# Lainshower/debiasing-multi-modal

Hardware: AMD Instinct MI355X
Metric: images/sec (embed+adapter step), CLIP-RN50 224px bs=1024 (higher is better)
Workload: dtype f32; 1 GPU; CLIP-RN50 224px encode_image + adapter(1024-128-1024) CE/SGD step, 1024 images/GPU, global batch 1024 (the metric's configuration, CLIP-RN50 224px bs=1024 on one GPU); global_batch=1024, batch_per_gpu=1024, parallelism=dp1, collective=none

## Files before the change

### debiasing-multi-modal_amd/_lib.py

```python
import ctypes
import glob
import os
import subprocess
from ctypes import c_double, c_float, c_int, c_int64, c_size_t, c_void_p

_HERE = os.path.dirname(os.path.abspath(__file__))
CSRC = os.path.join(_HERE, "csrc")
LIB_PATH = os.environ.get("DBMM_LIB") or os.path.join(_HERE, "libdbmm_hip.so")
INCLUDE = os.path.join(os.path.dirname(_HERE), "include")

_lib = None


def sources():
    return sorted(glob.glob(os.path.join(CSRC, "*.hip")))


KERNEL_SOURCES = (
    ("igemm_", ("igemm_f32.hip", "igemm_epilogue.inc", "common.h")),
    ("bottleneck_chain_kernel", ("bottleneck_chain.hip", "common.h")),
    ("bottleneck_chain8_kernel", ("bottleneck_chain8.hip", "common.h")),
    ("conv3x3_c32_kernel", ("conv_patch.hip", "common.h")),
    ("gemm_pair_8ph_kernel", ("gemm_pair_8ph.hip", "gemm_pair_8ph_epilogue.inc", "persistent_tiles.h", "common.h")),
    ("conv3x3_halo8", ("conv3x3_halo8.hip", "conv3x3_halo8_epilogue.inc", "persistent_tiles.h", "common.h")),
# ... 101 lines not shown
    "dbmm_bottleneck_chain_pool_f16": [_P, _P, _P, _P, _P, _P, _P, _P, _P, _P, _P, _L, _L, _L, _L, _L, _L, _P],
    "dbmm_bottleneck_chain_dual_f16": [_P, _P, _P, _P, _P, _P, _P, _P, _P, _P, _P, _P, _L, _L, _L, _L, _L, _P],
    "dbmm_conv3x3_bn_relu_f16": [_P, _P, _P, _P, _P, _L, _L, _L, _L, _L, _I, _P],
    "dbmm_conv_stem_s2_f16": [_P, _I, _P, _P, _P, _L, _L, _L, _L, _P],
    "dbmm_conv1x1_res_pool_f16": [_P, _P, _P, _P, _P, _P, _P, _L, _L, _L, _L, _L, _P],
    "dbmm_conv_stem_s2_bn_f16": [_P, _I, _P, _P, _P, _P, _L, _L, _L, _L, _P],
    "dbmm_avgpool2_f16": [_P, _P, _L, _L, _L, _L, _P],
    "dbmm_im2col_patch_f16": [_P, _I, _P, _L, _L, _L, _L, _P],
    "dbmm_vit_tokens_f16": [_P, _P, _P, _P, _L, _L, _L, _P],
    "dbmm_embed_gather_f16": [_P, _P, _P, _P, _L, _L, _L, _L, _P],
    "dbmm_gather_eot_f16": [_P, _P, _P, _L, _L, _L, _P],
    "dbmm_cast_f32_f16": [_P, _P, _L, _P],
    "dbmm_conv3x3_c32_bn_relu_x2": [_P, _P, _P, _I, _P, _P, _P, _P, _L, _L, _L, _L, _L, _I, _P],
    "dbmm_bottleneck_block_chain_x2": [_P, _P, _P, _I, _P, _P, _P, _I, _P, _P, _P, _P, _P, _P, _P, _P, _P, _P, _I, _P, _P, _P, _P,
                                       _L, _L, _L, _L, _L, _L, _P],
    "dbmm_gemm_bias_act_x3": [_P, _L, _P, _P, _L, _P, _P, _L, _P, _L, _L, _L, _L, _F, _I, _P, _Z, _P],
    "dbmm_gemm_batched": [_P, _L, _L, _I, _P, _L, _L, _I, _P, _L, _P, _L, _L, _L, _L, _L, _L, _F, _I, _P],
    "dbmm_gemm_pair_8ph": [_P, _L, _P, _P, _I, _L, _P, _P, _P, _L, _P, _L, _P, _L, _L, _L, _F, _I, _P],
    "dbmm_conv_stem_s2": [_P, _P, _P, _P, _P, _L, _L, _L, _L, _P],
    "dbmm_avgpool2d": [_P, _P, _L, _L, _L, _L, _L, _P],
    "dbmm_workspace_bytes_attnpool": [_L, _L, _L],
    "dbmm_attnpool": [_P, _P, _P, _P, _P, _P, _P, _P, _P, _L, _L, _L, _L, _L, _P, _Z, _P],
    "dbmm_attnpool_x": [_P, _I, _P, _P, _P, _P, _P, _P, _P, _P, _L, _L, _L, _L, _L, _P, _Z, _P],
    "dbmm_layernorm": [_P, _L, _P, _P, _P, _L, _L, _L, _F, _P, _P],
    "dbmm_mha_core": [_P, _P, _L, _L, _L, _L, _I, _P],
    "dbmm_mha_core_x2": [_P, _P, _P, _L, _L, _L, _L, _I, _P],
    "dbmm_embed_gather": [_P, _P, _P, _P, _L, _L, _L, _L, _P],
    "dbmm_im2col_patch": [_P, _P, _P, _L, _L, _L, _P],
    "dbmm_vit_tokens": [_P, _P, _P, _P, _L, _L, _L, _P],
    "dbmm_gather_eot": [_P, _P, _P, _L, _L, _L, _P],
# ... 147 lines not shown
```

### debiasing-multi-modal_amd/clip/model.py

```python
import os
import re
from collections import OrderedDict
from typing import Tuple, Union

import numpy as np
import torch
from torch import nn

from .. import ops



class _ConvW(nn.Module):
    def __init__(self, cin, cout, k):
        super().__init__()
        self.weight = nn.Parameter(torch.empty(cout, cin, k, k))


class _BNParams(nn.Module):
    def __init__(self, c):
        super().__init__()
        self.weight = nn.Parameter(torch.ones(c))
        self.bias = nn.Parameter(torch.zeros(c))
        self.register_buffer("running_mean", torch.zeros(c))
# ... 58 lines not shown

def _fold_bn(conv_w, bn):
    s = bn.weight.double() / torch.sqrt(bn.running_var.double() + bn.eps)
    w = conv_w.double() * s.reshape(-1, 1, 1, 1)
    b = bn.bias.double() - bn.running_mean.double() * s
    return w, b


def _conv_bn(conv, bn):
    w, b = _fold_bn(conv.weight, bn)
    scale = bn.weight.detach().double() / torch.sqrt(bn.running_var.detach().double() + bn.eps)
    return _pack_conv(w, b, raw=conv.weight.detach().float(), scale=scale)


_PLAN_OPTIONS = {"conv_split": ("f16", ("f16", "bf16", "off")), "conv_k_order": ("chunk32", ("chunk32", "tap")),
                 "fuse_ds": (1, (0, 1)), "fuse_chain": (1, (0, 1)), "fuse_conv2": (1, (0, 1)), "seam_pool": (2, (0, 1, 2))}
_opt = {}
_opt_version = [0]


def set_plan_option(name, value):
    default, allowed = _PLAN_OPTIONS[name]
    if isinstance(default, int):
        value = int(value)
    if value not in allowed:
        raise ValueError(f"plan option {name}: {value!r} not in {allowed}")
    old = _opt.get(name, default)
    _opt[name] = value
    _opt_version[0] += 1
    return old

# ... 240 lines not shown
                else:
                    out, oam = conv(x, am, e["c1"], None, 1, 0, ops.ACT_RELU)
                nxt = blocks[bi] if bi < len(blocks) else None
                if (e["stride"] == 1 and track and _opt["fuse_chain"] and _opt["fuse_conv2"] and nxt is not None and nxt["stride"] == 1
                        and all(c["sc"] is not None and c["ph"] is not None for c in (e["c2"], e["c3"], nxt["c1"]))
                        and ("ds" not in e or ("dual" in e and _opt["fuse_ds"]))):
                    ndsl = 3 if "ds" in e else 2
                    x_am, y1_am = amax[slot[0] + 1:slot[0] + 2], amax[slot[0] + ndsl:slot[0] + ndsl + 1]
                    dual = dict(a2=x, a2_absmax=am, ds=e["ds"], ratio=e["dual"]["ratio"], bias=e["dual"]["bias"]) if "ds" in e else None
                    r = ops.bottleneck_block_chain(out, oam, e["c2"], e["c3"], nxt["c1"], residual=None if dual else x, dual=dual,
                                                   x_absmax=x_am, y1n_absmax=y1_am)
                    if r is not None:
                        slot[0] += ndsl + 1
                        x, am, x_pooled, y1_next = r[0], x_am, None, (r[1], y1_am)
                        continue
                if e["stride"] == 2:
                    out, oam = conv(out, oam, e["c2"], None, 3, 1, ops.ACT_RELU, pool=2)
                else:
                    out, oam = conv(out, oam, e["c2"], None, 3, 1, ops.ACT_RELU)
                    if e["stride"] > 1:
                        out = ops.avgpool2d(out, e["stride"])
                identity = x
                fused = None
                if "ds" in e:
                    if e["stride"] > 1:
                        identity = x_pooled if (x_pooled is not None and e["stride"] == 2) else ops.avgpool2d(x, e["stride"])
                    nxt = blocks[bi] if bi < len(blocks) else None
                    if ("dual" in e and track and _opt["fuse_ds"] and _opt["fuse_chain"] and e["stride"] == 1 and nxt is not None
                            and nxt["c1"]["sc"] is not None and nxt["c1"]["ph"] is not None and "ds" not in nxt):
                        x_am, y1_am = amax[slot[0]:slot[0] + 1], amax[slot[0] + 2:slot[0] + 3]
# ... 325 lines not shown
```

### debiasing-multi-modal_amd/csrc/bottleneck_chain.hip

```cpp
#include <stdlib.h>
#include "common.h"

namespace {

struct ChainP {
    const float* a; const float* a_absmax;
    const u16* w3; int w3_exp; const float* sc3; const float* b3;
    const float* res; float* x; float* xp; float* x_absmax;
    const u16* w1; int w1_exp; const float* sc1; const float* b1;
    float* y1; float* y1_absmax;
    int M, N;
    int Ho, Wo;
    const float* a2; const float* a2_absmax; const u16* wd; const float* ratio;
    const u16* w2; int w2_exp; const float* sc2; const float* b2;
    int H, W;
};

template <int RH>
__device__ __forceinline__ int swz(int row) { return RH == 32 ? ((row >> 2) & 3) : (RH == 64 ? ((row >> 1) & 7) : (row & 15)); }

constexpr int BM = 128;

template <int K, int P>
struct ChainGeo {
    static constexpr int BNS = K == 64 ? 64 : 32;
    static constexpr int SLROW = BNS + 4;
    static constexpr int R1_BYTES = BM * SLROW * 4 > 2 * BM * 64 * 2 ? BM * SLROW * 4 : 2 * BM * 64 * 2;
    static constexpr int W3_BYTES = BNS * K * 2;
    static constexpr int W1_BYTES = P * BNS * 2;
    static constexpr int LDS_BYTES = R1_BYTES + W3_BYTES + W1_BYTES;
// ... 8 lines not shown
}

constexpr int C2_SROWS = 132, C2_PLANE = C2_SROWS * 32;
constexpr int C2_W2P = 104;
template <int K>
struct Conv2Geo {
    static constexpr int W2_OFF = 2 * C2_PLANE;
    static constexpr int GROUP_BYTES = (2 * C2_PLANE * 2 + K * C2_W2P * 2 + 255) / 256 * 256;
    static constexpr int NST = K == 64 ? 2 : 1;
    static constexpr int Z_OFF = NST * GROUP_BYTES;
    static constexpr int BYTES = Z_OFF + 256;
    static constexpr int STAGE_BYTES = BM * 68 * 4;
};
constexpr int cmax(int a, int b) { return a > b ? a : b; }

template <int K, int P, int POOL, int DUAL = 0, int CONV2 = 0>
__global__ __launch_bounds__(256, 2) void bottleneck_chain_kernel(const ChainP p) {
    static_assert(!DUAL || K == 64, "dual-source variant: layer-1 geometry (K = K2 = 64)");
    static_assert(!CONV2 || !POOL, "the conv2 phase walks pixels in standard order");
    static_assert(K == 64 || K == 128, "conv3 reduction depth: 64 (layer 1) or 128 (layer 2)");
    static_assert(P == 64 || P == 128, "conv1' width");
    using G = ChainGeo<K, P>;
    constexpr int BNS = G::BNS, SLROW = G::SLROW;
    constexpr int KS = K / 16, TN3 = BNS / 32, TN1 = P / 32;
    constexpr int LDS_TOTAL = cmax(G::LDS_BYTES + (DUAL ? BNS * 64 * 2 : 0), CONV2 ? cmax(Conv2Geo<K>::BYTES, Conv2Geo<K>::STAGE_BYTES) : 0);
    __shared__ __attribute__((aligned(256))) unsigned char lds_raw[LDS_TOTAL];
    u16* Ay = (u16*)lds_raw;
    float* slab = (float*)lds_raw;
    u16* W3b = (u16*)(lds_raw + G::R1_BYTES);
    u16* W1b = (u16*)(lds_raw + G::R1_BYTES + G::W3_BYTES);
    u16* Wdb = (u16*)(lds_raw + G::R1_BYTES + G::W3_BYTES + G::W1_BYTES);

    const int tid = threadIdx.x, lane = tid & 63, wave = tid >> 6;
    const int fr = lane & 31, fh = lane >> 5;
    const int m0 = xcd_remap(blockIdx.x, gridDim.x) * BM;
    const int NT = p.N / BNS;

    const int g0 = row_pixel<POOL>(p, m0);
    const long long Mll = p.M;
    const __amdgpu_buffer_rsrc_t rsA = desc(p.a, Mll * K * 4, (long long)g0 * K * 4);
    const __amdgpu_buffer_rsrc_t rsR = DUAL ? desc(p.a2, Mll * 64 * 4, (long long)g0 * 64 * 4)
                                            : desc(p.res, Mll * p.N * 4, (long long)g0 * p.N * 4);
    const __amdgpu_buffer_rsrc_t rsX = desc(p.x, POOL == 2 ? 0 : Mll * p.N * 4, (long long)g0 * p.N * 4);
    const __amdgpu_buffer_rsrc_t rsY = desc(p.y1, Mll * P * 4, (long long)g0 * P * 4);
    __amdgpu_buffer_rsrc_t rsXP = rsX;
    if constexpr (POOL) rsXP = desc(p.xp, (Mll >> 2) * p.N * 4, (long long)(m0 >> 2) * p.N * 4);

    unsigned gx[4], gy[4];
#pragma unroll
    for (int t = 0; t < 4; ++t) {
        const int m = m0 + wave * 32 + 8 * t + 4 * fh;
        const int dp = row_pixel<POOL>(p, m) - g0;
        gx[t] = m < p.M ? (unsigned)dp * (unsigned)(p.N * 4) + (unsigned)(fr * 4) : OOR;
        gy[t] = m < p.M ? (unsigned)dp * (unsigned)(P * 4) + (unsigned)(fr * 4) : OOR;
    }
    auto qpix = [&](int q) { return POOL ? (q >> 1) * p.Wo + (q & 1) : q; };

    constexpr int CPR3 = K / 8, RPP3 = 256 / CPR3, W3LD = BNS * CPR3 / 256;
    constexpr int CPR1 = BNS / 8, RPP1 = 256 / CPR1, W1LD = P * CPR1 / 256;
    static_assert(W3LD >= 1 && W1LD >= 1, "weight slabs smaller than one pass of the workgroup");
    const int wc3 = tid % CPR3, wr3 = tid / CPR3, wc1 = tid % CPR1, wr1 = tid / CPR1;
    u32x4 w3r[W3LD], w1r[W1LD], wdr[DUAL ? W3LD : 1];
    auto load_w = [&](int nt) {
#pragma unroll
        for (int j = 0; j < W3LD; ++j) {
            w3r[j] = *(const u32x4*)(p.w3 + (size_t)(nt * BNS + wr3 + RPP3 * j) * K + wc3 * 8);
            if constexpr (DUAL) wdr[j] = *(const u32x4*)(p.wd + (size_t)(nt * BNS + wr3 + RPP3 * j) * 64 + wc3 * 8);
        }
#pragma unroll
        for (int j = 0; j < W1LD; ++j)
            w1r[j] = *(const u32x4*)(p.w1 + (size_t)(wr1 + RPP1 * j) * p.N + nt * BNS + wc1 * 8);
    };
    auto store_w = [&]() {
#pragma unroll
        for (int j = 0; j < W3LD; ++j) {
            const int row = wr3 + RPP3 * j;
            *(u32x4*)(W3b + row * K + ((wc3 ^ swz<K>(row)) << 3)) = w3r[j];
// ... 11 lines not shown
        if constexpr (DUAL) return;
#pragma unroll
        for (int j = 0; j < TN3; ++j)
#pragma unroll
            for (int r = 0; r < 16; ++r)
                rr[j][r] = __builtin_bit_cast(float, __builtin_amdgcn_raw_buffer_load_b32(
                    rsR, gx[r >> 2], (unsigned)((nt * BNS + j * 32) * 4 + qpix(r & 3) * p.N * 4), 0));
    };
    load_res(0);
    u32x4 af[KS][2], af2[DUAL ? 4 : 1][2];
    bool first_pass = true;
    auto stage_issue = [&](const __amdgpu_buffer_rsrc_t& rs, int ldk, int k0, f32x4 (&q)[8]) {
        const int lc = tid & 15, lr = tid >> 4;
#pragma unroll
        for (int i = 0; i < 8; ++i) {
            const int row = lr + 16 * i, m = m0 + row;
            const unsigned off = m < p.M ? (unsigned)(row_pixel<POOL>(p, m) - g0) * (unsigned)(ldk * 4) + lc * 16u : OOR;
            q[i] = __builtin_bit_cast(f32x4, __builtin_amdgcn_raw_buffer_load_b128(rs, off, (unsigned)(k0 * 4), 0));
        }
    };
    auto stage_finish = [&](const f32x4 (&q)[8], float sc, u32x4 (*dst)[2]) {
        const int lc = tid & 15, lr = tid >> 4;
        if (!first_pass) __syncthreads();
#pragma unroll
        for (int i = 0; i < 8; ++i) {
            const int row = lr + 16 * i;
            unsigned hp[2], lp[2];
#pragma unroll
            for (int j = 0; j < 2; ++j) split2h_pair(q[i][2 * j], q[i][2 * j + 1], sc, hp[j], lp[j]);
            const int off = row * 64 + (((lc >> 1) ^ swz<64>(row)) << 3) + ((lc & 1) << 2);
            *(u32x2*)(Ay + off) = (u32x2){hp[0], hp[1]};
            *(u32x2*)(Ay + BM * 64 + off) = (u32x2){lp[0], lp[1]};
// ... 18 lines not shown
    if constexpr (DUAL && CONV2) stage_issue(rsR, 64, 0, q2);
    int s_a;
    if constexpr (!CONV2) {
        s_a = scale_exp(*p.a_absmax);
#pragma unroll
        for (int kp = 0; kp < K / 64; ++kp) stage_pass(rsA, K, kp * 64, pow2f(s_a), af + kp * 4);
    } else {
        using C2 = Conv2Geo<K>;
        constexpr int TN2 = K / 32, NG = (K / 32) * 3, W2LD = (K * 12 + 255) / 256;
        u16* Sp = (u16*)lds_raw;
        constexpr int NST = C2::NST, STH = C2::GROUP_BYTES / 2;
        constexpr int ZLH = C2::Z_OFF / 2;
        if (tid < 16) *(u32x4*)(lds_raw + C2::Z_OFF + tid * 16) = (u32x4){0u, 0u, 0u, 0u};
        const int s_y1 = scale_exp(*p.a_absmax);
        const float y1_sc = pow2f(s_y1);
        const int px0 = m0 - 1 - p.W > 0 ? m0 - 1 - p.W : 0;
        const __amdgpu_buffer_rsrc_t rsS = desc(p.a, Mll * K * 4, (long long)px0 * K * 4);
        const int lc = tid & 7, lr = tid >> 3;
        unsigned s_off[5];
#pragma unroll
        for (int i = 0; i < 5; ++i) {
            const int j = lr + 32 * i;
            s_off[i] = j < 130 ? (unsigned)((m0 - 1 + j - px0) * (K * 4)) + lc * 16u : OOR;
        }
        unsigned fmask = 0;
        {
            const int m = m0 + wave * 32 + fr;
            if (m < p.M) {
                const int hw = p.H * p.W, rem = m - (m / hw) * hw, ho = rem / p.W, wo = rem - ho * p.W;
#pragma unroll
                for (int kh = 0; kh < 3; ++kh)
#pragma unroll
                    for (int kw = 0; kw < 3; ++kw)
                        if (ho + kh - 1 >= 0 && ho + kh - 1 < p.H && wo + kw - 1 >= 0 && wo + kw - 1 < p.W) fmask |= 1u << (kh * 3 + kw);
            }
        }
        f32x4 sq[5];
        u32x4 w2q[W2LD];
        auto load_group = [&](int g) {
            const int sl = g / 3, kh = g - sl * 3;
            const unsigned delta = (unsigned)(((kh - 1) * p.W * K + sl * 32) * 4);
#pragma unroll
            for (int i = 0; i < 5; ++i)
// ... 26 lines not shown
            }
        };
        f32x16 acc2[TN2];
#pragma unroll
        for (int j = 0; j < TN2; ++j)
#pragma unroll
            for (int r = 0; r < 16; ++r) acc2[j][r] = 0.f;
        auto compute_group = [&](int g, int st) {
            const u16* Sps = Sp + st * STH;
            const u16* W2b = Sps + C2::W2_OFF;
            const int zl = ZLH - st * STH;
            const int kh = g % 3;
#pragma unroll
            for (int kw = 0; kw < 3; ++kw) {
                const bool ok = (fmask >> (kh * 3 + kw)) & 1u;
                const int row = wave * 32 + fr + kw;
#pragma unroll
                for (int ks = 0; ks < 2; ++ks) {
                    const int addr = row * 32 + (((2 * ks + fh) ^ swz<32>(row)) << 3);
                    const int a0 = ok ? addr : zl + (addr & 127), a1 = ok ? addr + C2_PLANE : zl + (addr & 127);
                    const u32x4 ah = *(const u32x4*)(Sps + a0), al = *(const u32x4*)(Sps + a1);
                    u32x4 wf[TN2];
#pragma unroll
                    for (int j = 0; j < TN2; ++j) wf[j] = *(const u32x4*)(W2b + (j * 32 + fr) * C2_W2P + kw * 32 + (2 * ks + fh) * 8);
#pragma unroll
                    for (int j = 0; j < TN2; ++j)
                        acc2[j] = __builtin_amdgcn_mfma_f32_32x32x16_f16(__builtin_bit_cast(f16x8, al), __builtin_bit_cast(f16x8, wf[j]), acc2[j], 0, 0, 0);
#pragma unroll
                    for (int j = 0; j < TN2; ++j)
                        acc2[j] = __builtin_amdgcn_mfma_f32_32x32x16_f16(__builtin_bit_cast(f16x8, ah), __builtin_bit_cast(f16x8, wf[j]), acc2[j], 0, 0, 0);
                }
// ... 52 lines not shown
        }
        __syncthreads();
        if constexpr (!DUAL) store_w();
    }
    float dual_dyn = 1.f;
    if constexpr (DUAL) {
        const int s_a2 = scale_exp(*p.a2_absmax);
        if constexpr (CONV2) stage_finish(q2, pow2f(s_a2), af2);
        else stage_pass(rsR, 64, 0, pow2f(s_a2), af2);
        dual_dyn = pow2f(s_a - s_a2);
    }
    __syncthreads();

    float* Ls = slab + wave * (32 * SLROW);
    const float acc3_scale = pow2f(-s_a - p.w3_exp);
    f32x16 acc1[TN1];
#pragma unroll
    for (int j = 0; j < TN1; ++j)
#pragma unroll
        for (int r = 0; r < 16; ++r) acc1[j][r] = 0.f;
    float run_max = 0.f, x_amax = 0.f;
    int s_cur = 0;

    for (int nt = 0; nt < NT; ++nt) {
        const int n0 = nt * BNS;
        if (nt + 1 < NT) load_w(nt + 1);
        f32x16 acc3[TN3];
#pragma unroll
        for (int j = 0; j < TN3; ++j)
#pragma unroll
            for (int r = 0; r < 16; ++r) acc3[j][r] = 0.f;
// ... 37 lines not shown
        }
        float tmax = 0.f;
#pragma unroll
        for (int j = 0; j < TN3; ++j) {
            const int n = n0 + j * 32 + fr;
            const float sv = p.sc3[n] * acc3_scale, bv = p.b3[n];
#pragma unroll
            for (int r = 0; r < 16; ++r) {
                float v = fmaxf(fmaf(acc3[j][r], sv, bv) + (DUAL ? 0.f : rr[j][r]), 0.f);
                if (gx[r >> 2] == OOR) v = 0.f;
                acc3[j][r] = v;
                tmax = fmaxf(tmax, v);
                if constexpr (POOL != 2)
                    __builtin_amdgcn_raw_buffer_store_b32(__builtin_bit_cast(unsigned, v), rsX, gx[r >> 2],
                                                          (unsigned)((n0 + j * 32) * 4 + qpix(r & 3) * p.N * 4), 0);
                Ls[((r & 3) + 8 * (r >> 2) + 4 * fh) * SLROW + j * 32 + fr] = v;
            }
            if constexpr (POOL) {
#pragma unroll
                for (int t = 0; t < 4; ++t) {
                    const float s = (((acc3[j][4 * t] + acc3[j][4 * t + 1]) + acc3[j][4 * t + 2]) + acc3[j][4 * t + 3]) * 0.25f;
                    const int mp = wave * 8 + 2 * t + fh;
                    const unsigned off = gx[t] != OOR ? (unsigned)mp * (unsigned)(p.N * 4) + (unsigned)(fr * 4) : OOR;
                    __builtin_amdgcn_raw_buffer_store_b32(__builtin_bit_cast(unsigned, s), rsXP, off, (unsigned)((n0 + j * 32) * 4), 0);
                }
            }
        }
        if (nt + 1 < NT) load_res(nt + 1);
        tmax = wave_max(tmax);
        x_amax = fmaxf(x_amax, tmax);
        if (tmax > run_max) {
            run_max = tmax;
            const int s_new = scale_exp(run_max);
            if (s_new != s_cur) {
                const float f = pow2f(s_new - s_cur);
#pragma unroll
                for (int j = 0; j < TN1; ++j)
#pragma unroll
                    for (int r = 0; r < 16; ++r) acc1[j][r] *= f;
                s_cur = s_new;
            }
        }
        const float t_sc = pow2f(s_cur);
#pragma unroll
        for (int ks = 0; ks < BNS / 16; ++ks) {
            const f32x4 x0 = *(const f32x4*)(Ls + fr * SLROW + 16 * ks + 8 * fh);
            const f32x4 x1 = *(const f32x4*)(Ls + fr * SLROW + 16 * ks + 8 * fh + 4);
            unsigned h[4], l[4];
            split2h_pair(x0[0], x0[1], t_sc, h[0], l[0]); split2h_pair(x0[2], x0[3], t_sc, h[1], l[1]);
            split2h_pair(x1[0], x1[1], t_sc, h[2], l[2]); split2h_pair(x1[2], x1[3], t_sc, h[3], l[3]);
            const u32x4 ah = {h[0], h[1], h[2], h[3]}, al = {l[0], l[1], l[2], l[3]};
            u32x4 wf[TN1];
#pragma unroll
            for (int j = 0; j < TN1; ++j) {
                const int row = j * 32 + fr;
                wf[j] = *(const u32x4*)(W1b + row * BNS + (((2 * ks + fh) ^ swz<BNS>(row)) << 3));
            }
#pragma unroll
            for (int j = 0; j < TN1; ++j)
                acc1[j] = __builtin_amdgcn_mfma_f32_32x32x16_f16(__builtin_bit_cast(f16x8, al), __builtin_bit_cast(f16x8, wf[j]),
                                                                 acc1[j], 0, 0, 0);
#pragma unroll
            for (int j = 0; j < TN1; ++j)
                acc1[j] = __builtin_amdgcn_mfma_f32_32x32x16_f16(__builtin_bit_cast(f16x8, ah), __builtin_bit_cast(f16x8, wf[j]),
                                                                 acc1[j], 0, 0, 0);
        }
        __syncthreads();
// ... 57 lines not shown
        return DBMM_E_ALIGN;
    ChainP p{};
    p.a = y1; p.a_absmax = y1_absmax;
    p.w2 = (const u16*)w2_plane_f16; p.w2_exp = w2_exp; p.sc2 = scale2; p.b2 = bias2; p.H = (int)H; p.W = (int)W;
    p.w3 = (const u16*)w3_plane_f16; p.w3_exp = w3_exp; p.sc3 = scale3; p.b3 = bias3;
    p.res = residual; p.a2 = a2; p.a2_absmax = a2_absmax; p.wd = (const u16*)wd_plane_f16; p.ratio = ratio;
    p.x = x_out; p.x_absmax = x_absmax;
    p.w1 = (const u16*)w1_plane_f16; p.w1_exp = w1_exp; p.sc1 = scale1; p.b1 = bias1;
    p.y1 = y1_out; p.y1_absmax = y1_out_absmax;
    p.M = (int)M; p.N = (int)N; p.Ho = (int)H; p.Wo = (int)W;
    const dim3 grid((unsigned)((M + BM - 1) / BM));
    hipStream_t s = (hipStream_t)stream;
    if (dual) hipLaunchKernelGGL((bottleneck_chain_kernel<64, 64, 0, 1, 1>), grid, dim3(256), 0, s, p);
    else if (K == 64) hipLaunchKernelGGL((bottleneck_chain_kernel<64, 64, 0, 0, 1>), grid, dim3(256), 0, s, p);
    else hipLaunchKernelGGL((bottleneck_chain_kernel<128, 128, 0, 0, 1>), grid, dim3(256), 0, s, p);
    DBMM_CHECK_LAUNCH();
    return DBMM_OK;
}

extern "C" int dbmm_bottleneck_chain_dual_x2(const float* y2, const float* y2_absmax, const void* w3_plane_f16, int w3_exp,
                                             const float* scale3, const float* bias, const float* a2, const float* a2_absmax,
                                             const void* wd_plane_f16, const float* ratio, float* x_out, float* x_absmax,
                                             const void* w1_plane_f16, int w1_exp, const float* scale1, const float* bias1,
                                             float* y1_out, float* y1_absmax, int64_t M, int64_t K, int64_t K2, int64_t N,
                                             int64_t P, void* stream) {
    if (!y2 || !y2_absmax || !w3_plane_f16 || !scale3 || !bias || !a2 || !a2_absmax || !wd_plane_f16 || !ratio || !x_out ||
        !w1_plane_f16 || !scale1 || !bias1 || !y1_out)
        return DBMM_E_ARG;
    if (M <= 0 || K <= 0 || K2 <= 0 || N <= 0 || P <= 0 || M > (INT32_MAX >> 1)) return DBMM_E_SHAPE;
    if (K != 64 || K2 != 64 || (N % 64) != 0 || (P != 64 && P != 128) || (M & 3)) return DBMM_E_UNSUPPORTED;
// ... 70 lines not shown
```

### debiasing-multi-modal_amd/ops.py

```python
import ctypes
import math
import os

import numpy as np
import torch

from . import _lib
from ._lib import check, ptr, require_cuda, stream

ACT_NONE, ACT_RELU, ACT_QUICKGELU = 0, 1, 2


class DbmmUnsupported(_lib.DbmmError):
    """a wrapper's C entry answered DBMM_E_UNSUPPORTED (no kernel for this valid request)"""


def set_option(name, value):
    old = get_option(name)
    check(_lib.lib().dbmm_set_option(name.encode(), int(value)), f"set_option({name})")
    return old


def get_option(name):
    v = ctypes.c_int()
# ... 369 lines not shown
    t.__enter__()
    d = dual or {}
    bias3 = d["bias"] if dual is not None else c3["b"]
    rc = _lib.lib().dbmm_bottleneck_block_chain_x2(
        ptr(y1), ptr(y1_absmax), ptr(c2["ph"]), int(c2["we"]), ptr(c2["sc"]), ptr(c2["b"]), ptr(c3["ph"]), int(c3["we"]),
        ptr(c3["sc"]), ptr(bias3), ptr(residual) if dual is None else None, ptr(d.get("a2")), ptr(d.get("a2_absmax")),
        ptr(d["ds"]["ph"]) if dual is not None else None, ptr(d.get("ratio")), ptr(x), ptr(x_absmax), ptr(c1["ph"]), int(c1["we"]),
        ptr(c1["sc"]), ptr(c1["b"]), ptr(y1n), ptr(y1n_absmax), B, H, W, K, N, P, stream())
    if rc == _lib.E_UNSUPPORTED:
        return None
    check(rc, "bottleneck_block_chain_x2")
    t.__exit__(None, None, None)
    return x, y1n


def bottleneck_chain_dual(y2, y2_absmax, c3, a2, a2_absmax, ds, ratio, bias, c1, x_absmax=None, y1_absmax=None):
    require_cuda(y2, a2)
    _f32c(y2); _f32c(a2)
    K, K2 = y2.shape[-1], a2.shape[-1]
    N, P = c3["ph"].shape[1], c1["ph"].shape[1]
    M = y2.numel() // K
    if (c3["ph"].shape[0] != 1 or ds["ph"].shape[0] != 1 or c1["ph"].shape[0] != 1 or a2.numel() // K2 != M
            or K != 64 or K2 != 64 or N % 64 or P not in (64, 128) or M % 4):
        return None
    x = _empty(tuple(y2.shape[:-1]) + (N,), device=y2.device, dtype=torch.float32)
    y1 = _empty(tuple(y2.shape[:-1]) + (P,), device=y2.device, dtype=torch.float32)
    global _chain_tag
    _chain_tag = f"bottleneck_chain_kernel<{K}, {P}, 0, 1>"
    t = _Timed(M, N, K + K2 + P, -1, 0, 4 * (M * K + M * K2 + M * N + M * P) + 2 * (N * K + N * K2 + P * N))
    t.__enter__()
# ... 1470 lines not shown
```

### include/dbmm.h

```cpp
#ifndef DBMM_H
#define DBMM_H

#include <stddef.h>
#include <stdint.h>

#ifdef __cplusplus
extern "C" {
#endif

#define DBMM_OK 0
#define DBMM_E_SHAPE (-1)
#define DBMM_E_ALIGN (-2)
#define DBMM_E_WORKSPACE (-3)
#define DBMM_E_ARG (-4)
#define DBMM_E_UNSUPPORTED (-5)

#define DBMM_WL_TAP_MAJOR 0
#define DBMM_WL_CHUNK_MAJOR 1
#define DBMM_WL_CHUNK32_MAJOR 2

#define DBMM_ACT_NONE 0
#define DBMM_ACT_RELU 1
#define DBMM_ACT_QUICKGELU 2

// ... 74 lines not shown

int dbmm_bottleneck_chain_dual_x2(const float* y2, const float* y2_absmax, const void* w3_plane_f16, int w3_exp,
                                  const float* scale3, const float* bias, const float* a2, const float* a2_absmax,
                                  const void* wd_plane_f16, const float* ratio, float* x_out, float* x_absmax,
                                  const void* w1_plane_f16, int w1_exp, const float* scale1, const float* bias1,
                                  float* y1_out, float* y1_absmax, int64_t M, int64_t K, int64_t K2, int64_t N,
                                  int64_t P, void* stream);

int dbmm_bottleneck_block_chain_x2(const float* y1, const float* y1_absmax, const void* w2_plane_f16, int w2_exp,
                                   const float* scale2, const float* bias2, const void* w3_plane_f16, int w3_exp,
                                   const float* scale3, const float* bias3, const float* residual, const float* a2,
                                   const float* a2_absmax, const void* wd_plane_f16, const float* ratio, float* x_out,
                                   float* x_absmax, const void* w1_plane_f16, int w1_exp, const float* scale1,
                                   const float* bias1, float* y1_out, float* y1_out_absmax, int64_t B, int64_t H,
                                   int64_t W, int64_t K, int64_t N, int64_t P, void* stream);

int dbmm_gemm_pair_8ph(const float* a, int64_t lda, const float* a_absmax, const void* w_plane_f16, int w_exp, int64_t ldw,
                       const float* out_scale, const float* bias, const float* residual, int64_t ldr, float* c, int64_t ldc,
                       float* c_absmax, int64_t M, int64_t N, int64_t K, float alpha, int act, void* stream);

int dbmm_gemm_f16(const void* a, int64_t lda, const void* w, int64_t ldw, const float* bias, const void* residual,
                  int64_t ldr, void* c, int64_t ldc, int64_t M, int64_t N, int64_t K, int act, void* stream);
int dbmm_gemm_f16_ws(const void* a, int64_t lda, const void* w, int64_t ldw, const float* bias, const void* residual,
                     int64_t ldr, void* c, int64_t ldc, int64_t M, int64_t N, int64_t K, int act, void* workspace,
                     size_t workspace_bytes, void* stream);
int dbmm_conv1x1_bn_act_f16(const void* x, const void* w, const float* scale, const float* bias, const void* residual, void* y,
                            int64_t M, int64_t Cin, int64_t Cout, int act, void* stream);
int dbmm_conv1x1_dual_bn_act_f16(const void* y2, const void* w3, const float* scale3, const void* xp, const void* wd, const float* ratio,
                                 const float* bias, void* out, int64_t M, int64_t K, int64_t K2, int64_t Cout, int act, void* stream);
int dbmm_bottleneck_chain_f16(const void* y2, const void* w3, const float* scale3, const float* bias3, const void* residual, void* x_out,
// ... 326 lines not shown
```

Baseline: 36740 images/sec.

## Fuse conv2+conv3 of last stride-1 block before downsample stage via row-tiled chain

Adds a ROWT row-tile mode to the bottleneck chain kernel, so a workgroup covers whole image rows and walks pixels in 2x2-window order. The conv2 3x3 phase can then run alongside the pooled output. Two new entry points use it for the last stride-1 block before a stride-2 stage. The tail variant (enabled by default) fuses conv2, conv3, residual add and the 2x2 pooled copy into one launch. The seam variant (off by default) also fuses the next block's conv1. The aim is to remove separate conv2 launches and the round-trips of intermediate activations and pooled tensors through memory. The cost is more kernel template variants and tiles sized by image rows, which can leave workgroups partly filled.

Measured after the change: 36910 images/sec (median of 6 runs). No clear change (+0.4%).

```diff
diff --git a/debiasing-multi-modal_amd/_lib.py b/debiasing-multi-modal_amd/_lib.py
--- a/debiasing-multi-modal_amd/_lib.py
+++ b/debiasing-multi-modal_amd/_lib.py
@@ -139,6 +139,9 @@
     "dbmm_conv3x3_c32_bn_relu_x2": [_P, _P, _P, _I, _P, _P, _P, _P, _L, _L, _L, _L, _L, _I, _P],
     "dbmm_bottleneck_block_chain_x2": [_P, _P, _P, _I, _P, _P, _P, _I, _P, _P, _P, _P, _P, _P, _P, _P, _P, _P, _I, _P, _P, _P, _P,
                                        _L, _L, _L, _L, _L, _L, _P],
+    "dbmm_bottleneck_block_chain_pool_x2": [_P, _P, _P, _I, _P, _P, _P, _I, _P, _P, _P, _P, _P, _P, _I, _P, _P, _P, _P,
+                                            _L, _L, _L, _L, _L, _L, _P],
+    "dbmm_bottleneck_block_tail_x2": [_P, _P, _P, _I, _P, _P, _P, _I, _P, _P, _P, _P, _P, _P, _L, _L, _L, _L, _L, _P],
     "dbmm_gemm_bias_act_x3": [_P, _L, _P, _P, _L, _P, _P, _L, _P, _L, _L, _L, _L, _F, _I, _P, _Z, _P],
     "dbmm_gemm_batched": [_P, _L, _L, _I, _P, _L, _L, _I, _P, _L, _P, _L, _L, _L, _L, _L, _L, _F, _I, _P],
     "dbmm_gemm_pair_8ph": [_P, _L, _P, _P, _I, _L, _P, _P, _P, _L, _P, _L, _P, _L, _L, _L, _F, _I, _P],
diff --git a/debiasing-multi-modal_amd/clip/model.py b/debiasing-multi-modal_amd/clip/model.py
--- a/debiasing-multi-modal_amd/clip/model.py
+++ b/debiasing-multi-modal_amd/clip/model.py
@@ -96,7 +96,8 @@
 
 
 _PLAN_OPTIONS = {"conv_split": ("f16", ("f16", "bf16", "off")), "conv_k_order": ("chunk32", ("chunk32", "tap")),
-                 "fuse_ds": (1, (0, 1)), "fuse_chain": (1, (0, 1)), "fuse_conv2": (1, (0, 1)), "seam_pool": (2, (0, 1, 2))}
+                 "fuse_ds": (1, (0, 1)), "fuse_chain": (1, (0, 1)), "fuse_conv2": (1, (0, 1)), "seam_pool": (2, (0, 1, 2)),
+                 "seam_conv2": (0, (0, 1)), "tail_conv2": (1, (0, 1))}
 _opt = {}
 _opt_version = [0]
 
@@ -367,6 +368,23 @@
                         slot[0] += ndsl + 1
                         x, am, x_pooled, y1_next = r[0], x_am, None, (r[1], y1_am)
                         continue
+                if (e["stride"] == 1 and track and _opt["fuse_chain"] and _opt["fuse_conv2"] and "ds" not in e and nxt is not None
+                        and nxt["stride"] == 2 and "ds" in nxt and all(c["sc"] is not None and c["ph"] is not None for c in (e["c2"], e["c3"]))):
+                    x_am = amax[slot[0] + 1:slot[0] + 2]
+                    if (_opt["seam_conv2"] and _opt["seam_pool"] == 2 and not return_stages and nxt["c1"]["sc"] is not None
+                            and nxt["c1"]["ph"] is not None):
+                        y1_am = amax[slot[0] + 2:slot[0] + 3]
+                        r = ops.bottleneck_block_chain_pool(out, oam, e["c2"], e["c3"], nxt["c1"], x, x_am, y1_am)
+                        if r is not None:
+                            slot[0] += 3
+                            x, am, x_pooled, y1_next = None, x_am, r[0], (r[1], y1_am)
+                            continue
+                    if _opt["tail_conv2"]:
+                        r = ops.bottleneck_block_tail(out, oam, e["c2"], e["c3"], x, x_am)
+                        if r is not None:
+                            slot[0] += 2
+                            (x, x_pooled), am = r, x_am
+                            continue
                 if e["stride"] == 2:
                     out, oam = conv(out, oam, e["c2"], None, 3, 1, ops.ACT_RELU, pool=2)
                 else:
diff --git a/debiasing-multi-modal_amd/csrc/bottleneck_chain.hip b/debiasing-multi-modal_amd/csrc/bottleneck_chain.hip
--- a/debiasing-multi-modal_amd/csrc/bottleneck_chain.hip
+++ b/debiasing-multi-modal_amd/csrc/bottleneck_chain.hip
@@ -14,6 +14,7 @@
     const float* a2; const float* a2_absmax; const u16* wd; const float* ratio;
     const u16* w2; int w2_exp; const float* sc2; const float* b2;
     int H, W;
+    int R;
 };
 
 template <int RH>
@@ -52,12 +53,13 @@
 };
 constexpr int cmax(int a, int b) { return a > b ? a : b; }
 
-template <int K, int P, int POOL, int DUAL = 0, int CONV2 = 0>
+template <int K, int P, int POOL, int DUAL = 0, int CONV2 = 0, int ROWT = 0>
 __global__ __launch_bounds__(256, 2) void bottleneck_chain_kernel(const ChainP p) {
     static_assert(!DUAL || K == 64, "dual-source variant: layer-1 geometry (K = K2 = 64)");
-    static_assert(!CONV2 || !POOL, "the conv2 phase walks pixels in standard order");
+    static_assert(!CONV2 || !POOL || ROWT, "the conv2 phase walks pixels in standard order");
+    static_assert(!ROWT || (CONV2 && POOL && !DUAL), "row tiles: the pooled launches that start at conv2");
     static_assert(K == 64 || K == 128, "conv3 reduction depth: 64 (layer 1) or 128 (layer 2)");
-    static_assert(P == 64 || P == 128, "conv1' width");
+    static_assert(P == 64 || P == 128 || (P == 0 && POOL == 1), "conv1' width (0: none, x' and its pooled copy are the outputs)");
     using G = ChainGeo<K, P>;
     constexpr int BNS = G::BNS, SLROW = G::SLROW;
     constexpr int KS = K / 16, TN3 = BNS / 32, TN1 = P / 32;
@@ -71,10 +73,21 @@
 
     const int tid = threadIdx.x, lane = tid & 63, wave = tid >> 6;
     const int fr = lane & 31, fh = lane >> 5;
-    const int m0 = xcd_remap(blockIdx.x, gridDim.x) * BM;
+    const int tile = xcd_remap(blockIdx.x, gridDim.x);
+    const int m0 = tile * BM;
+    const int RW = ROWT ? p.R * p.W : BM;
     const int NT = p.N / BNS;
-
-    const int g0 = row_pixel<POOL>(p, m0);
+    auto row_live = [&](int ml) { return ROWT ? ml < RW : m0 + ml < p.M; };
+
+    const int g0 = ROWT ? tile * RW : row_pixel<POOL>(p, m0);
+    auto row_off = [&](int ml) {
+        if constexpr (ROWT) {
+            const int win = ml >> 2, wp2 = p.W >> 1, wr = win / wp2;
+            return (2 * wr + ((ml >> 1) & 1)) * p.W + 2 * (win - wr * wp2) + (ml & 1);
+        } else {
+            return row_pixel<POOL>(p, m0 + ml) - g0;
+        }
+    };
     const long long Mll = p.M;
     const __amdgpu_buffer_rsrc_t rsA = desc(p.a, Mll * K * 4, (long long)g0 * K * 4);
     const __amdgpu_buffer_rsrc_t rsR = DUAL ? desc(p.a2, Mll * 64 * 4, (long long)g0 * 64 * 4)
@@ -82,23 +95,24 @@
     const __amdgpu_buffer_rsrc_t rsX = desc(p.x, POOL == 2 ? 0 : Mll * p.N * 4, (long long)g0 * p.N * 4);
     const __amdgpu_buffer_rsrc_t rsY = desc(p.y1, Mll * P * 4, (long long)g0 * P * 4);
     __amdgpu_buffer_rsrc_t rsXP = rsX;
-    if constexpr (POOL) rsXP = desc(p.xp, (Mll >> 2) * p.N * 4, (long long)(m0 >> 2) * p.N * 4);
+    if constexpr (POOL) rsXP = desc(p.xp, (Mll >> 2) * p.N * 4, (long long)((ROWT ? g0 : m0) >> 2) * p.N * 4);
 
     unsigned gx[4], gy[4];
 #pragma unroll
     for (int t = 0; t < 4; ++t) {
-        const int m = m0 + wave * 32 + 8 * t + 4 * fh;
-        const int dp = row_pixel<POOL>(p, m) - g0;
-        gx[t] = m < p.M ? (unsigned)dp * (unsigned)(p.N * 4) + (unsigned)(fr * 4) : OOR;
-        gy[t] = m < p.M ? (unsigned)dp * (unsigned)(P * 4) + (unsigned)(fr * 4) : OOR;
+        const int ml = wave * 32 + 8 * t + 4 * fh;
+        const bool live = row_live(ml);
+        const int dp = row_off(ml);
+        gx[t] = live ? (unsigned)dp * (unsigned)(p.N * 4) + (unsigned)(fr * 4) : OOR;
+        gy[t] = live ? (unsigned)dp * (unsigned)(P * 4) + (unsigned)(fr * 4) : OOR;
     }
     auto qpix = [&](int q) { return POOL ? (q >> 1) * p.Wo + (q & 1) : q; };
 
     constexpr int CPR3 = K / 8, RPP3 = 256 / CPR3, W3LD = BNS * CPR3 / 256;
     constexpr int CPR1 = BNS / 8, RPP1 = 256 / CPR1, W1LD = P * CPR1 / 256;
-    static_assert(W3LD >= 1 && W1LD >= 1, "weight slabs smaller than one pass of the workgroup");
+    static_assert(W3LD >= 1 && (W1LD >= 1 || P == 0), "weight slabs smaller than one pass of the workgroup");
     const int wc3 = tid % CPR3, wr3 = tid / CPR3, wc1 = tid % CPR1, wr1 = tid / CPR1;
-    u32x4 w3r[W3LD], w1r[W1LD], wdr[DUAL ? W3LD : 1];
+    u32x4 w3r[W3LD], w1r[W1LD ? W1LD : 1], wdr[DUAL ? W3LD : 1];
     auto load_w = [&](int nt) {
 #pragma unroll
         for (int j = 0; j < W3LD; ++j) {
@@ -140,8 +154,8 @@
         const int lc = tid & 15, lr = tid >> 4;
 #pragma unroll
         for (int i = 0; i < 8; ++i) {
-            const int row = lr + 16 * i, m = m0 + row;
-            const unsigned off = m < p.M ? (unsigned)(row_pixel<POOL>(p, m) - g0) * (unsigned)(ldk * 4) + lc * 16u : OOR;
+            const int row = lr + 16 * i;
+            const unsigned off = row_live(row) ? (unsigned)row_off(row) * (unsigned)(ldk * 4) + lc * 16u : OOR;
             q[i] = __builtin_bit_cast(f32x4, __builtin_amdgcn_raw_buffer_load_b128(rs, off, (unsigned)(k0 * 4), 0));
         }
     };
@@ -190,19 +204,22 @@
         if (tid < 16) *(u32x4*)(lds_raw + C2::Z_OFF + tid * 16) = (u32x4){0u, 0u, 0u, 0u};
         const int s_y1 = scale_exp(*p.a_absmax);
         const float y1_sc = pow2f(s_y1);
-        const int px0 = m0 - 1 - p.W > 0 ? m0 - 1 - p.W : 0;
+        const int px0 = g0 - 1 - p.W > 0 ? g0 - 1 - p.W : 0;
         const __amdgpu_buffer_rsrc_t rsS = desc(p.a, Mll * K * 4, (long long)px0 * K * 4);
         const int lc = tid & 7, lr = tid >> 3;
         unsigned s_off[5];
 #pragma unroll
         for (int i = 0; i < 5; ++i) {
             const int j = lr + 32 * i;
-            s_off[i] = j < 130 ? (unsigned)((m0 - 1 + j - px0) * (K * 4)) + lc * 16u : OOR;
+            s_off[i] = j < RW + 2 ? (unsigned)((g0 - 1 + j - px0) * (K * 4)) + lc * 16u : OOR;
         }
         unsigned fmask = 0;
+        int c2row = wave * 32 + fr;
         {
-            const int m = m0 + wave * 32 + fr;
-            if (m < p.M) {
+            const bool live = row_live(c2row);
+            if constexpr (ROWT) c2row = live ? row_off(c2row) : 0;
+            const int m = g0 + c2row;
+            if (live) {
                 const int hw = p.H * p.W, rem = m - (m / hw) * hw, ho = rem / p.W, wo = rem - ho * p.W;
 #pragma unroll
                 for (int kh = 0; kh < 3; ++kh)
@@ -259,7 +276,7 @@
 #pragma unroll
             for (int kw = 0; kw < 3; ++kw) {
                 const bool ok = (fmask >> (kh * 3 + kw)) & 1u;
-                const int row = wave * 32 + fr + kw;
+                const int row = c2row + kw;
 #pragma unroll
                 for (int ks = 0; ks < 2; ++ks) {
                     const int addr = row * 32 + (((2 * ks + fh) ^ swz<32>(row)) << 3);
@@ -342,7 +359,7 @@
 
     float* Ls = slab + wave * (32 * SLROW);
     const float acc3_scale = pow2f(-s_a - p.w3_exp);
-    f32x16 acc1[TN1];
+    f32x16 acc1[TN1 ? TN1 : 1];
 #pragma unroll
     for (int j = 0; j < TN1; ++j)
 #pragma unroll
@@ -410,7 +427,7 @@
                 if constexpr (POOL != 2)
                     __builtin_amdgcn_raw_buffer_store_b32(__builtin_bit_cast(unsigned, v), rsX, gx[r >> 2],
                                                           (unsigned)((n0 + j * 32) * 4 + qpix(r & 3) * p.N * 4), 0);
-                Ls[((r & 3) + 8 * (r >> 2) + 4 * fh) * SLROW + j * 32 + fr] = v;
+                if constexpr (P != 0) Ls[((r & 3) + 8 * (r >> 2) + 4 * fh) * SLROW + j * 32 + fr] = v;
             }
             if constexpr (POOL) {
 #pragma unroll
@@ -439,14 +456,14 @@
         }
         const float t_sc = pow2f(s_cur);
 #pragma unroll
-        for (int ks = 0; ks < BNS / 16; ++ks) {
+        for (int ks = 0; ks < (P ? BNS / 16 : 0); ++ks) {
             const f32x4 x0 = *(const f32x4*)(Ls + fr * SLROW + 16 * ks + 8 * fh);
             const f32x4 x1 = *(const f32x4*)(Ls + fr * SLROW + 16 * ks + 8 * fh + 4);
             unsigned h[4], l[4];
             split2h_pair(x0[0], x0[1], t_sc, h[0], l[0]); split2h_pair(x0[2], x0[3], t_sc, h[1], l[1]);
             split2h_pair(x1[0], x1[1], t_sc, h[2], l[2]); split2h_pair(x1[2], x1[3], t_sc, h[3], l[3]);
             const u32x4 ah = {h[0], h[1], h[2], h[3]}, al = {l[0], l[1], l[2], l[3]};
-            u32x4 wf[TN1];
+            u32x4 wf[TN1 ? TN1 : 1];
 #pragma unroll
             for (int j = 0; j < TN1; ++j) {
                 const int row = j * 32 + fr;
@@ -534,6 +551,71 @@
     if (dual) hipLaunchKernelGGL((bottleneck_chain_kernel<64, 64, 0, 1, 1>), grid, dim3(256), 0, s, p);
     else if (K == 64) hipLaunchKernelGGL((bottleneck_chain_kernel<64, 64, 0, 0, 1>), grid, dim3(256), 0, s, p);
     else hipLaunchKernelGGL((bottleneck_chain_kernel<128, 128, 0, 0, 1>), grid, dim3(256), 0, s, p);
+    DBMM_CHECK_LAUNCH();
+    return DBMM_OK;
+}
+
+static int rowtile_rows(int64_t H, int64_t W) {
+    if ((H & 1) || (W & 1) || 2 * W > BM) return 0;
+    for (int64_t R = (BM / W) & ~(int64_t)1; R >= 2; R -= 2)
+        if (H % R == 0) return (int)R;
+    return 0;
+}
+
+extern "C" int dbmm_bottleneck_block_chain_pool_x2(const float* y1, const float* y1_absmax, const void* w2_plane_f16, int w2_exp,
+                                                   const float* scale2, const float* bias2, const void* w3_plane_f16, int w3_exp,
+                                                   const float* scale3, const float* bias3, const float* residual, float* x_pooled,
+                                                   float* x_absmax, const void* w1_plane_f16, int w1_exp, const float* scale1,
+                                                   const float* bias1, float* y1_out, float* y1_out_absmax, int64_t B, int64_t H,
+                                                   int64_t W, int64_t K, int64_t N, int64_t P, void* stream) {
+    if (!y1 || !y1_absmax || !w2_plane_f16 || !scale2 || !bias2 || !w3_plane_f16 || !scale3 || !bias3 || !residual || !x_pooled ||
+        !w1_plane_f16 || !scale1 || !bias1 || !y1_out)
+        return DBMM_E_ARG;
+    if (B <= 0 || H <= 0 || W <= 0 || K <= 0 || N <= 0 || P <= 0) return DBMM_E_SHAPE;
+    const int64_t M = B * H * W;
+    if (M > (INT32_MAX >> 1)) return DBMM_E_SHAPE;
+    const int R = rowtile_rows(H, W);
+    if (K != 64 || P != 128 || (N % 64) != 0 || (M & 3) || !R) return DBMM_E_UNSUPPORTED;
+    if (w2_exp < -40 || w2_exp > 40 || w3_exp < -40 || w3_exp > 40 || w1_exp < -40 || w1_exp > 40) return DBMM_E_UNSUPPORTED;
+    if (!dbmm_aligned16(y1) || !dbmm_aligned16(w2_plane_f16) || !dbmm_aligned16(w3_plane_f16) || !dbmm_aligned16(w1_plane_f16) ||
+        !dbmm_aligned16(residual) || !dbmm_aligned16(x_pooled) || !dbmm_aligned16(y1_out))
+        return DBMM_E_ALIGN;
+    ChainP p{};
+    p.a = y1; p.a_absmax = y1_absmax;
+    p.w2 = (const u16*)w2_plane_f16; p.w2_exp = w2_exp; p.sc2 = scale2; p.b2 = bias2; p.H = (int)H; p.W = (int)W; p.R = R;
+    p.w3 = (const u16*)w3_plane_f16; p.w3_exp = w3_exp; p.sc3 = scale3; p.b3 = bias3;
+    p.res = residual; p.xp = x_pooled; p.x_absmax = x_absmax;
+    p.w1 = (const u16*)w1_plane_f16; p.w1_exp = w1_exp; p.sc1 = scale1; p.b1 = bias1;
+    p.y1 = y1_out; p.y1_absmax = y1_out_absmax;
+    p.M = (int)M; p.N = (int)N; p.Ho = (int)H; p.Wo = (int)W;
+    hipLaunchKernelGGL((bottleneck_chain_kernel<64, 128, 2, 0, 1, 1>), dim3((unsigned)(B * (H / R))), dim3(256), 0, (hipStream_t)stream, p);
+    DBMM_CHECK_LAUNCH();
+    return DBMM_OK;
+}
+
+extern "C" int dbmm_bottleneck_block_tail_x2(const float* y1, const float* y1_absmax, const void* w2_plane_f16, int w2_exp,
+                                             const float* scale2, const float* bias2, const void* w3_plane_f16, int w3_exp,
+                                             const float* scale3, const float* bias3, const float* residual, float* x_out,
+                                             float* x_pooled, float* x_absmax, int64_t B, int64_t H, int64_t W, int64_t K, int64_t N,
+                                             void* stream) {
+    if (!y1 || !y1_absmax || !w2_plane_f16 || !scale2 || !bias2 || !w3_plane_f16 || !scale3 || !bias3 || !residual || !x_out || !x_pooled)
+        return DBMM_E_ARG;
+    if (B <= 0 || H <= 0 || W <= 0 || K <= 0 || N <= 0) return DBMM_E_SHAPE;
+    const int64_t M = B * H * W;
+    if (M > (INT32_MAX >> 1)) return DBMM_E_SHAPE;
+    const int R = rowtile_rows(H, W);
+    if (K != 128 || (N % 64) != 0 || (M & 3) || !R) return DBMM_E_UNSUPPORTED;
+    if (w2_exp < -40 || w2_exp > 40 || w3_exp < -40 || w3_exp > 40) return DBMM_E_UNSUPPORTED;
+    if (!dbmm_aligned16(y1) || !dbmm_aligned16(w2_plane_f16) || !dbmm_aligned16(w3_plane_f16) || !dbmm_aligned16(residual) ||
+        !dbmm_aligned16(x_out) || !dbmm_aligned16(x_pooled))
+        return DBMM_E_ALIGN;
+    ChainP p{};
+    p.a = y1; p.a_absmax = y1_absmax;
+    p.w2 = (const u16*)w2_plane_f16; p.w2_exp = w2_exp; p.sc2 = scale2; p.b2 = bias2; p.H = (int)H; p.W = (int)W; p.R = R;
+    p.w3 = (const u16*)w3_plane_f16; p.w3_exp = w3_exp; p.sc3 = scale3; p.b3 = bias3;
+    p.res = residual; p.x = x_out; p.xp = x_pooled; p.x_absmax = x_absmax;
+    p.M = (int)M; p.N = (int)N; p.Ho = (int)H; p.Wo = (int)W;
+    hipLaunchKernelGGL((bottleneck_chain_kernel<128, 0, 1, 0, 1, 1>), dim3((unsigned)(B * (H / R))), dim3(256), 0, (hipStream_t)stream, p);
     DBMM_CHECK_LAUNCH();
     return DBMM_OK;
 }
diff --git a/debiasing-multi-modal_amd/ops.py b/debiasing-multi-modal_amd/ops.py
--- a/debiasing-multi-modal_amd/ops.py
+++ b/debiasing-multi-modal_amd/ops.py
@@ -407,6 +407,68 @@
     return x, y1n
 
 
+def _block_operands(y1, c2, c3, residual):
+    require_cuda(y1, residual)
+    _f32c(y1); _f32c(residual)
+    B, H, W, K = y1.shape
+    N = c3["ph"].shape[1]
+    if (c2["ph"] is None or c2["ph"].shape[0] != 1 or c2["wl"] != WL_CHUNK32_MAJOR or tuple(c2["ph"].shape[1:]) != (K, 9 * K)
+            or c3["ph"].shape[0] != 1 or N % 64 or (B * H * W) % 4 or tuple(residual.shape) != (B, H, W, N)):
+        return None
+    return B, H, W, K, N
+
+
+def bottleneck_block_chain_pool(y1, y1_absmax, c2, c3, c1, residual, x_absmax=None, y1n_absmax=None):
+    shp = _block_operands(y1, c2, c3, residual)
+    if shp is None or c1["ph"].shape[0] != 1:
+        return None
+    B, H, W, K, N = shp
+    P = c1["ph"].shape[1]
+    if (K, P) != (64, 128) or H % 2 or W % 2:
+        return None
+    M = B * H * W
+    xp = _empty((B, H // 2, W // 2, N), device=y1.device, dtype=torch.float32)
+    y1n = _empty((B, H, W, P), device=y1.device, dtype=torch.float32)
+    global _chain_tag
+    _chain_tag = f"bottleneck_chain_kernel<{K}, {P}, 2, 0, 1, 1>"
+    nby = 4 * (M * K + M * N + M // 4 * N + M * P) + 2 * (K * 9 * K + N * K + P * N)
+    t = _Timed(M, 1, 9 * K * K + N * (K + P), -1, 0, nby)
+    t.__enter__()
+    rc = _lib.lib().dbmm_bottleneck_block_chain_pool_x2(
+        ptr(y1), ptr(y1_absmax), ptr(c2["ph"]), int(c2["we"]), ptr(c2["sc"]), ptr(c2["b"]), ptr(c3["ph"]), int(c3["we"]),
+        ptr(c3["sc"]), ptr(c3["b"]), ptr(residual), ptr(xp), ptr(x_absmax), ptr(c1["ph"]), int(c1["we"]), ptr(c1["sc"]),
+        ptr(c1["b"]), ptr(y1n), ptr(y1n_absmax), B, H, W, K, N, P, stream())
+    if rc == _lib.E_UNSUPPORTED:
+        return None
+    check(rc, "bottleneck_block_chain_pool_x2")
+    t.__exit__(None, None, None)
+    return xp, y1n
+
+
+def bottleneck_block_tail(y1, y1_absmax, c2, c3, residual, x_absmax=None):
+    shp = _block_operands(y1, c2, c3, residual)
+    if shp is None:
+        return None
+    B, H, W, K, N = shp
+    if K != 128 or H % 2 or W % 2:
+        return None
+    M = B * H * W
+    x = _empty((B, H, W, N), device=y1.device, dtype=torch.float32)
+    xp = _empty((B, H // 2, W // 2, N), device=y1.device, dtype=torch.float32)
+    global _chain_tag
+    _chain_tag = f"bottleneck_chain_kernel<{K}, 0, 1, 0, 1, 1>"
+    t = _Timed(M, 1, 9 * K * K + N * K, -1, 0, 4 * (M * K + 2 * M * N + M // 4 * N) + 2 * (K * 9 * K + N * K))
+    t.__enter__()
+    rc = _lib.lib().dbmm_bottleneck_block_tail_x2(
+        ptr(y1), ptr(y1_absmax), ptr(c2["ph"]), int(c2["we"]), ptr(c2["sc"]), ptr(c2["b"]), ptr(c3["ph"]), int(c3["we"]),
+        ptr(c3["sc"]), ptr(c3["b"]), ptr(residual), ptr(x), ptr(xp), ptr(x_absmax), B, H, W, K, N, stream())
+    if rc == _lib.E_UNSUPPORTED:
+        return None
+    check(rc, "bottleneck_block_tail_x2")
+    t.__exit__(None, None, None)
+    return x, xp
+
+
 def bottleneck_chain_dual(y2, y2_absmax, c3, a2, a2_absmax, ds, ratio, bias, c1, x_absmax=None, y1_absmax=None):
     require_cuda(y2, a2)
     _f32c(y2); _f32c(a2)
diff --git a/include/dbmm.h b/include/dbmm.h
--- a/include/dbmm.h
+++ b/include/dbmm.h
@@ -112,6 +112,18 @@
                                    float* x_absmax, const void* w1_plane_f16, int w1_exp, const float* scale1,
                                    const float* bias1, float* y1_out, float* y1_out_absmax, int64_t B, int64_t H,
                                    int64_t W, int64_t K, int64_t N, int64_t P, void* stream);
+
+int dbmm_bottleneck_block_chain_pool_x2(const float* y1, const float* y1_absmax, const void* w2_plane_f16, int w2_exp,
+                                        const float* scale2, const float* bias2, const void* w3_plane_f16, int w3_exp,
+                                        const float* scale3, const float* bias3, const float* residual, float* x_pooled,
+                                        float* x_absmax, const void* w1_plane_f16, int w1_exp, const float* scale1,
+                                        const float* bias1, float* y1_out, float* y1_out_absmax, int64_t B, int64_t H,
+                                        int64_t W, int64_t K, int64_t N, int64_t P, void* stream);
+int dbmm_bottleneck_block_tail_x2(const float* y1, const float* y1_absmax, const void* w2_plane_f16, int w2_exp,
+                                  const float* scale2, const float* bias2, const void* w3_plane_f16, int w3_exp,
+                                  const float* scale3, const float* bias3, const float* residual, float* x_out,
+                                  float* x_pooled, float* x_absmax, int64_t B, int64_t H, int64_t W, int64_t K, int64_t N,
+                                  void* stream);
 
 int dbmm_gemm_pair_8ph(const float* a, int64_t lda, const float* a_absmax, const void* w_plane_f16, int w_exp, int64_t ldw,
                        const float* out_scale, const float* bias, const float* residual, int64_t ldr, float* c, int64_t ldc,
```
